# nerfstudio-project/nerfstudio

Measured on AMD Instinct MI355X. Metric: training rays/sec (4096 rays x 48 samples per GPU), higher is better.
Workload: dtype f32

## Files before the change

nerfstudio_amd/csrc/field_mlp.hip:

```cpp

#include "common.h"
#include "field_reduce.h"
#include "launch.h"
#include "mfma_chain.h"
#include "scatter.h"
#include "wave.h"

NSAMD_PROBE_DEFINE(field)

namespace nsamd {

constexpr int kWaves = 4;
constexpr int kFieldThreads = 64 * kWaves;
constexpr int kScratchLd = 20;
constexpr int kScratchTile = 64 * kScratchLd;

template <int NT, int KT, int THREADS>
__device__ __forceinline__ void stage_frag_load(float* v, const float* __restrict__ W, int n_real, int k_real, bool head0,
                                                int app_dim) {
  static_assert(THREADS % 256 == 0 && (NT * KT * 256) % THREADS == 0, "whole tiles per pass");
  const int r = threadIdx.x & 3, lane = (threadIdx.x >> 2) & 63;
  const int j = lane & 15, g = lane >> 4;
#pragma unroll
  for (int i = 0; i < NT * KT * 256 / THREADS; ++i) {
// ... 135 lines not shown
  stage_frag_load<4, 2, THREADS>(v, mlp.base_W0, 64, 32, false, 0);
  stage_frag_load<1, 4, THREADS>(v + 2 * U, mlp.base_W1, 16, 64, false, 0);
  stage_frag_load<4, 4, THREADS>(v + 3 * U, mlp.head_W0, 64, 31 + app_dim, true, app_dim);
  stage_frag_load<4, 4, THREADS>(v + 7 * U, mlp.head_W1, 64, 64, false, 0);
  stage_frag_load<1, 4, THREADS>(v + 11 * U, mlp.head_W2, 3, 64, false, 0);
  stage_frag_store<4, 2, THREADS>(wf + kOffBase0, v);
  stage_frag_store<1, 4, THREADS>(wf + kOffBase1, v + 2 * U);
  stage_frag_store<4, 4, THREADS>(wf + kOffHead0, v + 3 * U);
  stage_frag_store<4, 4, THREADS>(wf + kOffHead1, v + 7 * U);
  stage_frag_store<1, 4, THREADS>(wf + kOffHead2, v + 11 * U);
  stage_bias<THREADS>(bias + kBiasBase0, mlp.base_b0, 64, 64);
  stage_bias<THREADS>(bias + kBiasBase1, mlp.base_b1, 16, 16);
  stage_bias<THREADS>(bias + kBiasHead0, mlp.head_b0, 64, 64);
  stage_bias<THREADS>(bias + kBiasHead1, mlp.head_b1, 64, 64);
  stage_bias<THREADS>(bias + kBiasHead2, mlp.head_b2, 3, 16);
}

template <int WAVES, bool RAYC = false>
__global__ __launch_bounds__(64 * WAVES, WAVES == 16 ? 1 : 2) void field_mlp_fwd_kernel(
    const float* __restrict__ enc, const float* __restrict__ selector, const float* __restrict__ directions,
    const int64_t* __restrict__ cams, const float* __restrict__ app_const, int64_t dir_group, int64_t M,
    nsamd_field_mlp mlp, int app_dim, float* __restrict__ density, float* __restrict__ rgb) {
  extern __shared__ __attribute__((aligned(16))) float lds[];
  float* wf = lds;
  float* bias = lds + kFragTotal;
  PROBE_STAMP(WAVES, 0);
  stage_all_fwd<64 * WAVES>(wf, bias, mlp, app_dim);
  __syncthreads();
  PROBE_STAMP(WAVES, 1);
  const int lane = threadIdx.x & 63, wave = threadIdx.x >> 6;
  const int64_t tiles = (M + 15) / 16;
  const float* app_table = cams ? mlp.appearance : nullptr;
  int probe_it = 0;
  for (int64_t tile = (int64_t)blockIdx.x * WAVES + wave; tile < tiles; tile += (int64_t)gridDim.x * WAVES) {
    asm volatile("" ::: "memory");
    const TileInputs ti = tile_inputs(tile, lane, M, selector, cams, dir_group);
    FieldActs A;
    load_enc_tile_fwd(enc, M, ti.p, lane, A.enc);
    if (RAYC && rgb != nullptr) {
      const float* c = mlp.ray_terms + ti.ray * 64 + 4 * (lane >> 4);
#pragma unroll
      for (int n = 0; n < 4; ++n) A.ha[n] = *reinterpret_cast<const v4f*>(c + 16 * n);
    }
    PROBE_STAMP(WAVES, 2 + 4 * probe_it);
    field_forward_tile<RAYC>(wf, bias, directions, app_table, app_const, dir_group, M, app_dim, ti, lane, A, 3 + 4 * probe_it,
                             rgb == nullptr);
    PROBE_STAMP(WAVES, 4 + 4 * probe_it);
    if (rgb != nullptr && mlp.saved_hb != nullptr && ti.live) {
#pragma unroll
      for (int t = 0; t < 4; ++t) *reinterpret_cast<v4f*>(mlp.saved_hb + ((tile * 4 + t) * 64 + lane) * 4) = A.hb[t];
    }
    if (lane < 16 && ti.live) {
      density[ti.p] = mlp.average_init_density * expf(A.o16[0][0]) * ti.sel;
      if (rgb != nullptr) {
        float* o = rgb + 3 * ti.p;
#pragma unroll
        for (int c = 0; c < 3; ++c) o[c] = 1.0f / (1.0f + expf(-A.rgbp[0][c]));
      }
    }
    PROBE_STAMP(WAVES, 5 + 4 * probe_it);
    ++probe_it;
  }
  PROBE_STAMP(WAVES, 63);
}

__global__ __launch_bounds__(kFieldThreads) void field_ray_terms_kernel(
    const float* __restrict__ directions, const int64_t* __restrict__ cams, const float* __restrict__ app_const,
    int64_t num_rays, nsamd_field_mlp mlp, int app_dim, float* __restrict__ terms, float* __restrict__ inputs,
    const float* __restrict__ slot_dev, int32_t slots) {
  __shared__ __attribute__((aligned(16))) float wf[kFragHead0];
  __shared__ __attribute__((aligned(16))) float bias[64];
  if (slot_dev != nullptr) {
    int32_t slot = (int32_t)slot_dev[0];
    slot = slot < 0 ? 0 : (slot >= slots ? slots - 1 : slot);
    directions += (int64_t)slot * 3 * num_rays;
    if (cams != nullptr) cams += (int64_t)slot * num_rays;
  }
  {
    float v[16];
    stage_frag_load<4, 4, kFieldThreads>(v, mlp.head_W0, 64, 31 + app_dim, true, app_dim);
    stage_frag_store<4, 4, kFieldThreads>(wf, v);
    stage_bias<kFieldThreads>(bias, mlp.head_b0, 64, 64);
  }
  __syncthreads();
  const int lane = threadIdx.x & 63, wave = threadIdx.x >> 6;
  const int j = lane & 15, g = lane >> 4;
  const float* app_table = cams ? mlp.appearance : nullptr;
  const int64_t tiles = (num_rays + 15) / 16;
  for (int64_t tile = (int64_t)blockIdx.x * kWaves + wave; tile < tiles; tile += (int64_t)gridDim.x * kWaves) {
    const int64_t ray = tile * 16 + j;
    const bool live = ray < num_rays;
    const int64_t rc = live ? ray : num_rays - 1;
    const float* d = directions + 3 * rc;
    v4f hin[4];
    hin[0] = sh_quad(d[0], d[1], d[2], g);
    if (app_dim > 0) {
      const float* src = (app_table != nullptr) ? app_table + cams[rc] * 32 : app_const;
      hin[2] = *reinterpret_cast<const v4f*>(src + 4 * g);
      hin[3] = *reinterpret_cast<const v4f*>(src + 16 + 4 * g);
    } else {
      hin[2] = v4f{0.f, 0.f, 0.f, 0.f};
      hin[3] = v4f{0.f, 0.f, 0.f, 0.f};
    }
    v4f acc[4];
    load_bias<4>(bias, acc, g);
    chain_gemm_tile<4, 4>(wf, 0, hin[0], acc, lane);
    chain_gemm_tile<4, 4>(wf, 2, hin[2], acc, lane);
    chain_gemm_tile<4, 4>(wf, 3, hin[3], acc, lane);
    if (live) {
#pragma unroll
      for (int n = 0; n < 4; ++n) *reinterpret_cast<v4f*>(terms + ray * 64 + 16 * n + 4 * g) = acc[n];
      if (inputs != nullptr) {
        float* x = inputs + ray * (16 + app_dim);
        *reinterpret_cast<v4f*>(x + 4 * g) = hin[0];
        if (app_dim > 0) {
          *reinterpret_cast<v4f*>(x + 16 + 4 * g) = hin[2];
          *reinterpret_cast<v4f*>(x + 32 + 4 * g) = hin[3];
        }
      }
    }
  }
}

typedef __bf16 bf16x8 __attribute__((ext_vector_type(8)));
typedef __bf16 bf16x2 __attribute__((ext_vector_type(2)));
typedef unsigned u4 __attribute__((ext_vector_type(4)));

__device__ __forceinline__ v4f mfma_bf16(const u4& a, const u4& b, v4f c) {
  return __builtin_amdgcn_mfma_f32_16x16x32_bf16(__builtin_bit_cast(bf16x8, a), __builtin_bit_cast(bf16x8, b), c, 0, 0, 0);
}

__device__ __forceinline__ unsigned pack_bf16(float a, float b) {
  bf16x2 p;
  p[0] = (__bf16)a;
  p[1] = (__bf16)b;
  return __builtin_bit_cast(unsigned, p);
}

__global__ void probe_mfma_bf16_kernel(const float* __restrict__ A, const float* __restrict__ B, float* __restrict__ out) {
  const int lane = threadIdx.x, j = lane & 15, g = lane >> 4;
  u4 a, b;
#pragma unroll
  for (int q = 0; q < 4; ++q) {
    a[q] = pack_bf16(A[j * 32 + 8 * g + 2 * q], A[j * 32 + 8 * g + 2 * q + 1]);
    b[q] = pack_bf16(B[(8 * g + 2 * q) * 16 + j], B[(8 * g + 2 * q + 1) * 16 + j]);
  }
  v4f c = {0.f, 0.f, 0.f, 0.f};
  c = mfma_bf16(a, b, c);
#pragma unroll
  for (int r = 0; r < 4; ++r) out[(4 * g + r) * 16 + j] = c[r];
}

__device__ __forceinline__ void split_pair(float x0, float x1, unsigned& o0, unsigned& o1) {
  const unsigned hh = pack_bf16(x0, x1);
  const float r0 = x0 - __uint_as_float(hh << 16);
  const float r1 = x1 - __uint_as_float(hh & 0xffff0000u);
  o0 = pack_bf16(r0, x0);
  o1 = pack_bf16(r1, x1);
}

template <int T>
__device__ __forceinline__ void store_rows_f32(float* S, const v4f* x, int j, int g) {
#pragma unroll
  for (int t = 0; t < T; ++t)
#pragma unroll
    for (int r = 0; r < 4; ++r) S[(16 * t + 4 * g + r) * kScratchLd + j] = x[t][r];
}

template <int T>
__device__ __forceinline__ void store_rows_pk(float* S, const v4f* x, int j, int g) {
  unsigned* U = reinterpret_cast<unsigned*>(S);
#pragma unroll
  for (int t = 0; t < T; ++t)
#pragma unroll
    for (int r = 0; r < 4; r += 2) {
      unsigned o0, o1;
      split_pair(x[t][r], x[t][r + 1], o0, o1);
      U[(16 * t + 4 * g + r) * kScratchLd + j] = o0;
      U[(16 * t + 4 * g + r + 1) * kScratchLd + j] = o1;
    }
}

template <int NT>
__device__ __forceinline__ void relu_mask(v4f* grad, const v4f* act) {
#pragma unroll
  for (int n = 0; n < NT; ++n)
#pragma unroll
    for (int r = 0; r < 4; ++r) grad[n][r] = (act[n][r] > 0.0f) ? grad[n][r] : 0.0f;
}

constexpr int kRayS = 16 * kScratchLd, kRayX = kRayS + 64;
constexpr int kCoopWaves = 8;
constexpr int kCoopThreads = 64 * kCoopWaves;
constexpr int kLd64 = 68, kLd32 = 36;
constexpr int kRowBase0 = 0, kRowBase1 = kRowBase0 + 64 * kLd32, kRowHead0 = kRowBase1 + 16 * kLd64,
              kRowHead1 = kRowHead0 + 64 * kLd64, kRowHead2 = kRowHead1 + 64 * kLd64,
              kRowTotal = kRowHead2 + 16 * kLd64;

template <int N_PAD, int K_PAD>
__device__ __forceinline__ void stage_rows_load(float* v, const float* __restrict__ W, int n_real, int k_real, bool head0,
                                                int app_dim) {
#pragma unroll
  for (int i = 0; i < N_PAD * K_PAD / kCoopThreads; ++i) {
    const int e = threadIdx.x + i * kCoopThreads;
    const int row = e / K_PAD, slot = e % K_PAD;
    const int col = head0 ? head0_col(slot, app_dim) : slot;
    v[i] = (row < n_real && col >= 0 && col < k_real) ? W[row * k_real + col] : 0.0f;
  }
}

template <int N_PAD, int K_PAD, int LD>
__device__ __forceinline__ void stage_rows_store(float* dst, const float* v) {
#pragma unroll
  for (int i = 0; i < N_PAD * K_PAD / kCoopThreads; ++i) {
    const int e = threadIdx.x + i * kCoopThreads;
    dst[(e / K_PAD) * LD + e % K_PAD] = v[i];
  }
}

template <int NT, int KT, int LD>
__device__ __forceinline__ void rows_gemm_fwd(const float* Wrows, const v4f* in, v4f* out, int j, int g) {
#pragma unroll
  for (int t = 0; t < KT; ++t) {
    v4f a[NT];
#pragma unroll
    for (int n = 0; n < NT; ++n) a[n] = *reinterpret_cast<const v4f*>(Wrows + (16 * n + j) * LD + 16 * t + 4 * g);
#pragma unroll
    for (int r = 0; r < 4; ++r) {
#pragma unroll
      for (int n = 0; n < NT; ++n) out[n] = mfma16(a[n][r], in[t][r], out[n]);
    }
  }
}

template <int MT, int NT, int LD>
__device__ __forceinline__ void rows_gemm_bwd(const float* Wrows, const v4f* in, v4f* out, int j, int g) {
#pragma unroll
  for (int t = 0; t < NT; ++t) {
    float a[4][MT];
#pragma unroll
    for (int r = 0; r < 4; ++r)
#pragma unroll
      for (int m = 0; m < MT; ++m) a[r][m] = Wrows[(16 * t + 4 * g + r) * LD + 16 * m + j];
#pragma unroll
    for (int r = 0; r < 4; ++r)
#pragma unroll
      for (int m = 0; m < MT; ++m) out[m] = mfma16(a[r][m], in[t][r], out[m]);
  }
}

template <int MT, int LD>
__device__ __forceinline__ void rows_gemm_bwd_rgb(const float* Wrows, float in_k, v4f* out, int j, int g) {
  float a[MT];
#pragma unroll
  for (int m = 0; m < MT; ++m) a[m] = Wrows[g * LD + 16 * m + j];
#pragma unroll
  for (int m = 0; m < MT; ++m) out[m] = mfma16(a[m], in_k, out[m]);
}

struct NoBetween {
  template <int I>
  __device__ __forceinline__ void at() const {}
};

template <class Between = NoBetween, bool RAYC = false, bool SAVED = false>
__device__ __forceinline__ void coop_forward_tile(const float* W, const float* bias, const float (&dir)[3],
                                                  const float* __restrict__ app_table,
                                                  const float* __restrict__ app_const, int app_dim,
                                                  const TileInputs& ti, int lane, FieldActs& A, const v4f* app_pre = nullptr,
                                                  const Between& between = Between(), const v4f* ray_terms = nullptr) {
  const int j = lane & 15, g = lane >> 4;
  load_bias<4>(bias + kBiasBase0, A.h1, g);
  rows_gemm_fwd<4, 2, kLd32>(W + kRowBase0, A.enc, A.h1, j, g);
  if (SAVED) {
    asm volatile("" : "+v"(A.hb[0]), "+v"(A.hb[1]), "+v"(A.hb[2]), "+v"(A.hb[3]), "+v"(A.sg[0]), "+v"(A.sg[1]), "+v"(A.sg[2]));
  }
  between.template at<0>();
  relu_tiles<4>(A.h1);
  load_bias<1>(bias + kBiasBase1, A.o16, g);
  rows_gemm_fwd<1, 4, kLd64>(W + kRowBase1, A.h1, A.o16, j, g);
  between.template at<1>();
  if (RAYC) {
#pragma unroll
    for (int n = 0; n < 4; ++n) A.ha[n] = ray_terms[n];
    rows_gemm_fwd<4, 1, kLd64>(W + kRowHead0 + 16, A.o16, A.ha, j, g);
  } else {
  A.hin[0] = sh_quad(dir[0], dir[1], dir[2], g);
  A.hin[1] = A.o16[0];
  if (app_pre != nullptr) {
    A.hin[2] = app_pre[0];
    A.hin[3] = app_pre[1];
  } else if (app_dim > 0) {
    const float* src = (app_table != nullptr) ? app_table + ti.cam * 32 : app_const;
    A.hin[2] = *reinterpret_cast<const v4f*>(src + 4 * g);
    A.hin[3] = *reinterpret_cast<const v4f*>(src + 16 + 4 * g);
  } else {
    A.hin[2] = v4f{0.f, 0.f, 0.f, 0.f};
    A.hin[3] = v4f{0.f, 0.f, 0.f, 0.f};
  }
  load_bias<4>(bias + kBiasHead0, A.ha, g);
  rows_gemm_fwd<4, 4, kLd64>(W + kRowHead0, A.hin, A.ha, j, g);
  }
  between.template at<2>();
  relu_tiles<4>(A.ha);
  if (!SAVED) {
    load_bias<4>(bias + kBiasHead1, A.hb, g);
    rows_gemm_fwd<4, 4, kLd64>(W + kRowHead1, A.ha, A.hb, j, g);
  }
  between.template at<3>();
  if (!SAVED) {
    relu_tiles<4>(A.hb);
    load_bias<1>(bias + kBiasHead2, A.rgbp, g);
    rows_gemm_fwd<1, 4, kLd64>(W + kRowHead2, A.hb, A.rgbp, j, g);
  }
  between.template at<4>();
}

__device__ __forceinline__ float dot2_ones(unsigned a, float c) {
  asm("v_dot2c_f32_bf16 %0, %1, %2" : "+v"(c) : "v"(a), "v"(0x3f803f80u));
  return c;
}

template <int TILES>
__device__ __forceinline__ void coop_dw_f32(v4f* acc, float* dbacc, bool want_db, const float* scratch, int first,
                                            int count, int n, int m0, int j, int g) {
#pragma unroll 2
  for (int area = first; area < first + count; ++area) {
    const float* Sd = scratch + area * 2 * kScratchTile;
    const float* Sx = Sd + kScratchTile;
    const v4f a = *reinterpret_cast<const v4f*>(Sd + (16 * n + j) * kScratchLd + 4 * g);
    v4f b[TILES];
#pragma unroll
    for (int i = 0; i < TILES; ++i) b[i] = *reinterpret_cast<const v4f*>(Sx + (16 * (m0 + i) + j) * kScratchLd + 4 * g);
    if (want_db) *dbacc += (a[0] + a[1]) + (a[2] + a[3]);
#pragma unroll
    for (int q = 0; q < 4; ++q)
#pragma unroll
      for (int i = 0; i < TILES; ++i) acc[i] = mfma16(a[q], b[i][q], acc[i]);
  }
}

template <int TILES>
__device__ __forceinline__ void coop_dw_pk(v4f* acc, float* dbacc, bool want_db, const float* scratch, int first,
                                           int count, int n, int m0, int j, int g) {
#pragma unroll 2
  for (int area = first; area < first + count; ++area) {
    const float* Sd = scratch + area * 2 * kScratchTile;
    const float* Sx = Sd + kScratchTile;
    const u4 a = *reinterpret_cast<const u4*>(Sd + (16 * n + j) * kScratchLd + 4 * g);
    u4 b[TILES];
#pragma unroll
    for (int i = 0; i < TILES; ++i) b[i] = *reinterpret_cast<const u4*>(Sx + (16 * (m0 + i) + j) * kScratchLd + 4 * g);
    if (want_db) {
      float s = *dbacc;
#pragma unroll
      for (int q = 0; q < 4; ++q) s = dot2_ones(a[q], s);
      *dbacc = s;
    }
    u4 ar;
#pragma unroll
    for (int q = 0; q < 4; ++q) ar[q] = __builtin_amdgcn_alignbit(a[q], a[q], 16);
#pragma unroll
    for (int i = 0; i < TILES; ++i) acc[i] = mfma_bf16(a, b[i], acc[i]);
#pragma unroll
    for (int i = 0; i < TILES; ++i) acc[i] = mfma_bf16(ar, b[i], acc[i]);
  }
}

template <int T, bool HEAD0 = false>
__device__ __forceinline__ void store_rows(float* S, const v4f* x, int j, int g) {
  if (HEAD0) store_rows_f32<T>(S, x, j, g);
  else store_rows_pk<T>(S, x, j, g);
}

template <int TILES, bool HEAD0 = false>
__device__ __forceinline__ void coop_dw(v4f* acc, float* dbacc, bool want_db, const float* scratch, int first,
                                        int count, int n, int m0, int j, int g) {
  if (HEAD0) coop_dw_f32<TILES>(acc, dbacc, want_db, scratch, first, count, n, m0, j, g);
  else coop_dw_pk<TILES>(acc, dbacc, want_db, scratch, first, count, n, m0, j, g);
}

__device__ __forceinline__ void coop_emit(const v4f& acc, int n, int m, int k_pad, float* partial_layer,
                                          float* __restrict__ dst, int n_real, int k_real, bool head0, int app_dim,
                                          int j, int g) {
#pragma unroll
  for (int r = 0; r < 4; ++r) {
    const int row = 16 * n + 4 * g + r, slot = 16 * m + j;
    if (partial_layer != nullptr) {
      partial_layer[row * k_pad + slot] = acc[r];
    } else if (dst != nullptr) {
      const int col = head0 ? head0_col(slot, app_dim) : slot;
      if (row < n_real && col >= 0 && col < k_real) unsafeAtomicAdd(dst + row * k_real + col, acc[r]);
    }
  }
}

__device__ __forceinline__ void coop_emit_bias(float v, int n, int j, int g, float* partial_bias, float* __restrict__ dst,
                                               int n_real) {
  v += __shfl_xor(v, 16);
  v += __shfl_xor(v, 32);
  if (g == 0) {
    if (partial_bias != nullptr) partial_bias[16 * n + j] = v;
    else if (dst != nullptr && 16 * n + j < n_real) unsafeAtomicAdd(dst + 16 * n + j, v);
  }
}


struct RouteArgs {
  nsamd_points P;
  int transform;
  nsamd_aabb box;
  nsamd_grid grid;
  ScatterGeom G;
  ScatterBufs buf;
};

constexpr int kProducerSegCap = 256;
constexpr int kRouteLevels = 16;
constexpr int kRouteCnt = kRouteLevels * (1 << kProducerMaxLog2Bins);

struct RouteLds {
  uint32_t cnt[kRouteCnt];
  struct Level {
    float scal;
    uint32_t loff;
    uint32_t lmax;
    uint32_t pad;
  } lv[kRouteLevels];
  nsamd_points P;
  nsamd_aabb box;
  int32_t transform, num_levels, log2_table_size, slice_log2, log2_bins;
  uint32_t seg_cap, static_end, level_cap, spill_cap, segs;
  uint4* queues;
  uint32_t* dyn_cursor;
  uint32_t* hdr;
  uint4* spill_rec;
  uint32_t* spill_tile;
  uint32_t* counts;
  float stash[kCoopWaves][11][64];
};
constexpr int kRouteLdsWords = (sizeof(RouteLds) + 3) / 4;
static_assert(sizeof(float) * (kRowTotal + 256 + kCoopWaves * 2 * kScratchTile) + sizeof(RouteLds) <= 160 * 1024, "160 KiB of LDS per CU");

__device__ __forceinline__ void route_lds_init(RouteLds* L, const RouteArgs& R) {
  for (int e = threadIdx.x; e < kRouteCnt; e += kCoopThreads) L->cnt[e] = 0u;
  if (threadIdx.x < kRouteLevels) {
    L->lv[threadIdx.x].scal = R.grid.scalings[threadIdx.x];
    L->lv[threadIdx.x].loff = R.G.level_off[threadIdx.x];
    L->lv[threadIdx.x].lmax = 0u;
    L->lv[threadIdx.x].pad = 0u;
  }
  if (threadIdx.x == 0) {
    L->P = R.P;
    L->box = R.box;
    L->transform = R.transform;
    L->num_levels = R.grid.num_levels;
    L->log2_table_size = R.grid.log2_table_size;
    L->slice_log2 = R.G.slice_log2;
    L->log2_bins = R.G.log2_bins;
    L->seg_cap = R.G.seg_cap;
    L->static_end = R.G.segs * R.G.seg_cap;
    L->level_cap = R.G.level_cap[0];
    L->spill_cap = R.G.spill_cap;
    L->segs = R.G.segs;
    L->queues = R.buf.queues;
    L->dyn_cursor = R.buf.dyn_cursor;
    L->hdr = R.buf.hdr;
    L->spill_rec = R.buf.spill_rec;
    L->spill_tile = R.buf.spill_tile;
    L->counts = R.buf.counts;
  }
}

__device__ __forceinline__ void route_spill(RouteLds* L, uint32_t tile, uint4 rec) {
  const uint32_t pos = atomicAdd(L->hdr + kHdrSpillCount, 1u);
  if (pos < L->spill_cap) {
    L->spill_rec[pos] = rec;
    L->spill_tile[pos] = tile;
  } else {
    atomicAdd(L->hdr + kHdrEvtLost, 1u);
  }
}


__device__ __noinline__ void route_record_slow(RouteLds* L, float x, float y, float z, float g0, float g1, int level, int q,
                                               bool segment_full) {
  const uint32_t mask = (1u << L->log2_table_size) - 1u;
  const int sl = L->slice_log2, lb = L->log2_bins;
  const uint32_t local_mask = (1u << sl) - 1u;
  const Cell c = locate_cell(x, y, z, L->lv[level].scal);
  const PairHash h = pair_hash(c, q, mask);
  const uint32_t bin = h.ia >> sl, tile0 = (uint32_t)level << lb;
  float a0, a1;
  pair_share(c, q, g0, g1, a0, a1);
  if ((h.ib >> sl) != bin) {
    const float omx = 1.0f - c.w[0];
    route_spill(L, tile0 + bin, single_record(a0 * omx, a1 * omx, h.ia & local_mask));
    route_spill(L, tile0 + (h.ib >> sl), single_record(a0 * c.w[0], a1 * c.w[0], h.ib & local_mask));
    return;
  }
  if (!segment_full) return;
  const uint4 rec = pair_record(a0, a1, c.w[0], h.ia & local_mask, h.ib & local_mask);
  const uint32_t Q = L->level_cap, static_end = L->static_end;
  const uint32_t pos = atomicAdd(L->dyn_cursor + (tile0 + bin), 1u);
  if (pos < Q - static_end) rec_store(L->queues + (L->lv[level].loff + bin * Q + static_end + pos), rec);
  else route_spill(L, tile0 + bin, rec);
}

template <int K>
__device__ __forceinline__ void route_level(RouteLds* L, const float (*stash)[64], int lane, uint32_t& gmax) {
  constexpr int t = K >> 1, rr = K & 1;
  const int g = lane >> 4;
  const int level = 8 * t + 2 * g + rr;
  const float g0 = stash[4 * t + 2 * rr][lane], g1 = stash[4 * t + 2 * rr + 1][lane];
  if (level >= L->num_levels || (g0 == 0.0f && g1 == 0.0f)) return;
  const float x = stash[8][lane], y = stash[9][lane], z = stash[10][lane];
  const Cell c = locate_cell(x, y, z, L->lv[level].scal);
  {
    const uint32_t b0 = __float_as_uint(g0) & 0x7fffffffu, b1 = __float_as_uint(g1) & 0x7fffffffu;
    gmax = max(gmax, max(b0, b1));
  }
  const uint32_t mask = (1u << L->log2_table_size) - 1u;
  const int sl = L->slice_log2;
  const uint32_t local_mask = (1u << sl) - 1u;
  const uint32_t C = L->seg_cap;
  uint32_t* const cnt = L->cnt + ((uint32_t)level << L->log2_bins);
  PairHash h[4];
  uint32_t rank[4];
#pragma unroll
  for (int q = 0; q < 4; ++q) h[q] = pair_hash(c, q, mask);
#pragma unroll
  for (int q = 0; q < 4; ++q)
    rank[q] = atomicAdd(cnt + (h[q].ia >> sl), 1u);
  uint4* const base = L->queues + (L->lv[level].loff + blockIdx.x * C);
  const uint32_t level_cap = L->level_cap;
  bool slow[4], full[4];
#pragma unroll
  for (int q = 0; q < 4; ++q) {
    const uint32_t bin = h[q].ia >> sl;
    const bool straddle = (h[q].ib >> sl) != bin;
    const float bz = (q & 2) ? c.w[2] : 1.0f - c.w[2];
    const float by = (q & 1) ? c.w[1] : 1.0f - c.w[1];
    const uint32_t a0 = straddle ? 0u : __float_as_uint((g0 * bz) * by), a1 = straddle ? 0u : __float_as_uint((g1 * bz) * by);
    const uint4 rec = pair_record(__uint_as_float(a0), __uint_as_float(a1), c.w[0], h[q].ia & local_mask,
                                  (straddle ? h[q].ia : h[q].ib) & local_mask);
    full[q] = rank[q] >= C;
    slow[q] = straddle || full[q];
    if (!full[q]) rec_store(base + (bin * level_cap + rank[q]), rec);
    full[q] = full[q] && !straddle;
  }
#pragma unroll
  for (int q = 0; q < 4; ++q)
    if (slow[q]) route_record_slow(L, x, y, z, g0, g1, level, q, full[q]);
}

__device__ __forceinline__ void route_flush(RouteLds* L, const float (*stash)[64], int lane, uint32_t (&gmax)[4]) {
  route_level<0>(L, stash, lane, gmax[0]);
  route_level<1>(L, stash, lane, gmax[1]);
  route_level<2>(L, stash, lane, gmax[2]);
  route_level<3>(L, stash, lane, gmax[3]);
}

__device__ __forceinline__ void route_publish_max(RouteLds* L, int lane, const uint32_t (&gmax)[4]) {
#pragma unroll
  for (int K = 0; K < 4; ++K) {
    const int level = 8 * (K >> 1) + 2 * (lane >> 4) + (K & 1);
    const uint32_t m = row16_max_u32(gmax[K]);
    if ((lane & 15) == 0 && level < L->num_levels && m != 0u) atomicMax(&L->lv[level].lmax, m);
  }
}

struct RawPosition {
  float o[3], d[3], t0, t1;
};

__device__ __forceinline__ bool route_ray_layout(const RouteLds* L, int64_t dir_group) {
  return L->P.positions == nullptr && (int64_t)L->P.samples_per_ray == dir_group;
}

__device__ __forceinline__ void route_issue_position(const RouteLds* L, int64_t tile, int64_t tiles, int64_t M,
                                                     int64_t dir_group, int lane, RawPosition& rp) {
  const int64_t pt = tile * 16 + (lane & 15);
  const bool rays = route_ray_layout(L, dir_group) && tile < tiles && pt < M;
  const int64_t p = rays ? pt : 0;
  const int64_t S = dir_group, ray = point_ray(p, S), s = p - ray * S;
  const NSAMD_GLOBAL_AS float* dummy = global_ptr(reinterpret_cast<const float*>(L->hdr));
  const NSAMD_GLOBAL_AS float* tb = rays ? global_ptr(L->P.t_bins) + ray * (S + 1) + s : dummy;
  const NSAMD_GLOBAL_AS float* o = rays ? global_ptr(L->P.origins) + 3 * ray : dummy;
  const NSAMD_GLOBAL_AS float* d = rays ? global_ptr(L->P.directions) + 3 * ray : dummy;
  rp.o[0] = o[0], rp.o[1] = o[1], rp.o[2] = o[2];
  rp.d[0] = d[0], rp.d[1] = d[1], rp.d[2] = d[2];
  rp.t0 = tb[0], rp.t1 = tb[1];
}

__device__ __forceinline__ bool route_finish_position(const RouteLds* L, const RawPosition& rp, int64_t tile, int64_t tiles,
                                                      int64_t M, int64_t dir_group, int lane, float& x, float& y, float& z) {
  const int64_t p = tile * 16 + (lane & 15);
  x = y = z = 0.0f;
  if (!(tile < tiles && p < M)) return false;
  if (!route_ray_layout(L, dir_group)) {
    load_position(L->P, p, x, y, z);
  } else {
    const float span = rp.t0 + rp.t1;
    x = rp.o[0] + rp.d[0] * span / 2.0f;
    y = rp.o[1] + rp.d[1] * span / 2.0f;
    z = rp.o[2] + rp.d[2] * span / 2.0f;
  }
  return true;
}

struct TileFetch {
  TileInputs ti;
  v4f enc[2];
  float up[4];
  float dir[3];
  v4f app[2];
  v4f cterm[4];
  float xin;
};

template <bool RAYC = false>
__device__ __forceinline__ void fetch_tile(TileFetch& f, int64_t tile, int64_t tiles, int lane, int64_t M,
                                           const float* __restrict__ enc, const float* __restrict__ selector,
                                           const float* __restrict__ directions, const int64_t* __restrict__ cams,
                                           const float* __restrict__ app_table, const float* __restrict__ app_const,
                                           int app_dim, int64_t dir_group, const float* __restrict__ ddensity,
                                           const float* __restrict__ drgb, const float* __restrict__ ray_terms = nullptr,
                                           const float* __restrict__ ray_inputs = nullptr) {
  const int g = lane >> 4;
  const int64_t t = tile < tiles ? tile : tiles - 1;
  const int64_t p = t * 16 + (lane & 15);
  f.ti.live = p < M && tile < tiles;
  f.ti.p = p < M ? p : M - 1;
  f.ti.ray = point_ray(f.ti.p, dir_group);
  if (RAYC) {
    f.ti.cam = 0;
  } else {
    const int64_t* cam_src = cams != nullptr ? cams + f.ti.ray : reinterpret_cast<const int64_t*>(enc);
    f.ti.cam = *cam_src;
  }
  f.ti.sel = (selector != nullptr ? selector : enc)[f.ti.p];
  load_enc_tile(enc, M, f.ti.p, lane, f.enc);
#define NSAMD_KEEP_APART() asm volatile("" ::: "memory")
  f.up[0] = drgb[3 * f.ti.p + 0];
  NSAMD_KEEP_APART();
  f.up[1] = drgb[3 * f.ti.p + 1];
  NSAMD_KEEP_APART();
  f.up[2] = drgb[3 * f.ti.p + 2];
  NSAMD_KEEP_APART();
  f.up[3] = ddensity[f.ti.p];
  if (RAYC) {
    const float* c = ray_terms + f.ti.ray * 64 + 4 * g;
#pragma unroll
    for (int n = 0; n < 4; ++n) f.cterm[n] = *reinterpret_cast<const v4f*>(c + 16 * n);
    const int ncols = 16 + app_dim;
    f.xin = ray_inputs[f.ti.ray * ncols + (lane < ncols ? lane : 0)];
    return;
  }
  const float* d = directions + 3 * f.ti.ray;
  f.dir[0] = d[0];
  NSAMD_KEEP_APART();
  f.dir[1] = d[1];
  NSAMD_KEEP_APART();
  f.dir[2] = d[2];
  NSAMD_KEEP_APART();
  const float* src = app_table != nullptr ? app_table + (cams != nullptr ? f.ti.cam : 0) * 32
                                          : (app_const != nullptr ? app_const : enc);
  f.app[0] = *reinterpret_cast<const v4f*>(src + 4 * g);
  f.app[1] = *reinterpret_cast<const v4f*>(src + 16 + 4 * g);
#undef NSAMD_KEEP_APART
}

struct RouteBetween {
  RouteLds* L;
  const float (*stash)[64];
  int lane;
  bool on;
  uint32_t* gmax;
  template <int I>
  __device__ __forceinline__ void at() const {
    if (!on) return;
    if (I == 0) route_level<0>(L, stash, lane, gmax[0]);
    if (I == 2) route_level<1>(L, stash, lane, gmax[1]);
  }
};

template <bool ROUTE, bool RAYC = false, bool SAVED = false>
__global__ __launch_bounds__(kCoopThreads) void field_mlp_bwd_kernel(
    const float* __restrict__ enc, const float* __restrict__ selector, const float* __restrict__ directions,
    const int64_t* __restrict__ cams, const float* __restrict__ app_const, int64_t dir_group, int64_t M,
    nsamd_field_mlp mlp, int app_dim, const float* __restrict__ ddensity, const float* __restrict__ drgb,
    float* __restrict__ denc, nsamd_field_mlp_grads grads, float* __restrict__ partials,
    float* __restrict__ app_partials, int app_rows_per_point, RouteArgs R) {
  extern __shared__ __attribute__((aligned(16))) float lds[];
  float* W = lds;
  float* bias = lds + kRowTotal;
  float* scratch = bias + 256;
  RouteLds* RL = reinterpret_cast<RouteLds*>(scratch + kCoopWaves * 2 * kScratchTile);
  if (ROUTE) route_lds_init(RL, R);
  PROBE_STAMP(kCoopWaves, 0);
  {
    float v[24];
    stage_rows_load<64, 32>(v, mlp.base_W0, 64, 32, false, 0);
    stage_rows_load<16, 64>(v + 4, mlp.base_W1, 16, 64, false, 0);
    stage_rows_load<64, 64>(v + 6, mlp.head_W0, 64, 31 + app_dim, true, app_dim);
    stage_rows_load<64, 64>(v + 14, mlp.head_W1, 64, 64, false, 0);
    stage_rows_load<16, 64>(v + 22, mlp.head_W2, 3, 64, false, 0);
    stage_rows_store<64, 32, kLd32>(W + kRowBase0, v);
    stage_rows_store<16, 64, kLd64>(W + kRowBase1, v + 4);
    stage_rows_store<64, 64, kLd64>(W + kRowHead0, v + 6);
    stage_rows_store<64, 64, kLd64>(W + kRowHead1, v + 14);
    stage_rows_store<16, 64, kLd64>(W + kRowHead2, v + 22);
  }
  for (int e = threadIdx.x; e < 256; e += kCoopThreads) {
    float v = 0.0f;
    if (e < kBiasBase1) v = mlp.base_b0[e];
    else if (e < kBiasHead0) v = mlp.base_b1[e - kBiasBase1];
    else if (e < kBiasHead1) v = mlp.head_b0[e - kBiasHead0];
    else if (e < kBiasHead2) v = mlp.head_b1[e - kBiasHead1];
    else if (e < kBiasHead2 + 3) v = mlp.head_b2[e - kBiasHead2];
    bias[e] = v;
  }
  __syncthreads();

  const int lane = threadIdx.x & 63, wave = threadIdx.x >> 6;
  const int j = lane & 15, g = lane >> 4;
  float* Sd = scratch + wave * 2 * kScratchTile;
  float* Sx = Sd + kScratchTile;
  const float* app_table = cams ? mlp.appearance : nullptr;
  const int own_n = wave >> 1;
  const int own_m2 = 2 * (wave & 1);
  const int own_m1 = wave & 1;
  const int own_q = wave & 3;
  const int own_half = wave >> 2;
  v4f dW_h1[2], dW_h0[2], dW_b0[1], dW_h2[1], dW_b1[1];
  v4f dW_r[2];
  zero_tiles<2>(dW_r);
  float db_h1 = 0.f, db_h0 = 0.f, db_b0 = 0.f, db_h2 = 0.f, db_b1 = 0.f;
// ... 50 lines not shown
    const bool emit = ROUTE && it > 0;
#define NSAMD_ROUTE_LEVEL(K)                                                      \
  do {                                                                           \
    if (ROUTE) {                                                                 \
      if (emit) route_level<K>(RL, RL->stash[wave], lane, route_gmax[K]); \
    }                                                                            \
  } while (0)

    v4f g_rgbp[1];
    zero_tiles<1>(g_rgbp);
    if (g == 0 && ti.live) {
#pragma unroll
      for (int c = 0; c < 3; ++c) {
        const float sg = SAVED ? A.sg[c] : 1.0f / (1.0f + expf(-A.rgbp[0][c]));
        g_rgbp[0][c] = up_rgb[c] * (sg * (1.0f - sg));
      }
    }
    float g_rgb_k;
    {
      const float s0 = __shfl(g_rgbp[0][0], j), s1 = __shfl(g_rgbp[0][1], j), s2 = __shfl(g_rgbp[0][2], j);
      g_rgb_k = g == 0 ? s0 : (g == 1 ? s1 : (g == 2 ? s2 : 0.0f));
    }
    __syncthreads();
    store_rows<1>(Sd, g_rgbp, j, g);
    store_rows<4>(Sx, A.hb, j, g);
    v4f g_hb[4];
    zero_tiles<4>(g_hb);
    rows_gemm_bwd_rgb<4, kLd64>(W + kRowHead2, g_rgb_k, g_hb, j, g);
    relu_mask<4>(g_hb, A.hb);
    __syncthreads();
    coop_dw<1>(dW_h2, &db_h2, bias_owner14, scratch, 4 * own_half, 4, 0, own_q, j, g);
    __syncthreads();
    PROBE_STAMP(kCoopWaves, 4 + 10 * (int)it);

    store_rows<4>(Sd, g_hb, j, g);
    store_rows<4>(Sx, A.ha, j, g);
    v4f g_ha[4];
    zero_tiles<4>(g_ha);
    rows_gemm_bwd<4, 4, kLd64>(W + kRowHead1, g_hb, g_ha, j, g);
    relu_mask<4>(g_ha, A.ha);
    NSAMD_ROUTE_LEVEL(2);
    __syncthreads();
    coop_dw<2>(dW_h1, &db_h1, bias_owner44, scratch, 0, kCoopWaves, own_n, own_m2, j, g);
    __syncthreads();
    PROBE_STAMP(kCoopWaves, 5 + 10 * (int)it);

    v4f g_hin[4];
    zero_tiles<4>(g_hin);
    if (RAYC) {
      store_rows<4>(Sd, g_ha, j, g);
      store_rows<1>(Sx, A.o16, j, g);
      rows_gemm_bwd<1, 4, kLd64>(W + kRowHead0 + 16, g_ha, g_hin + 1, j, g);
      float* Ss = Sx + kRayS;
#pragma unroll
      for (int n = 0; n < 4; ++n) {
        v4f v = g_ha[n];
#pragma unroll
        for (int r = 0; r < 4; ++r) v[r] = row16_sum_lane0(v[r]);
        if (j == 0) *reinterpret_cast<v4f*>(Ss + 16 * n + 4 * g) = v;
      }
      if (lane < 48) Sx[kRayX + lane] = lane < 16 + app_dim ? nxt_xin : 0.0f;
      __syncthreads();
      {
        coop_dw<1>(dW_h0, &db_h0, true, scratch, 4 * own_half, 4, own_q, 0, j, g);
        const int a = wave & 3, b0 = wave >> 2;
#pragma unroll
        for (int h = 0; h < 2; ++h) {
          const float* area = scratch + (4 * h + g) * 2 * kScratchTile + kScratchTile;
          const float sa = area[kRayS + 16 * a + j];
          if (b0 == 0 || app_dim > 0) dW_r[0] = mfma16(sa, area[kRayX + 16 * b0 + j], dW_r[0]);
          if (wave < 4 && app_dim > 0) dW_r[1] = mfma16(sa, area[kRayX + 32 + j], dW_r[1]);
        }
        if (wave < 2 && app_partials != nullptr) {
          v4f o = {0.f, 0.f, 0.f, 0.f};
          const float* st = scratch + (j & 7) * 2 * kScratchTile + kScratchTile + kRayS;
#pragma unroll
          for (int kk = 0; kk < 16; ++kk)
            o = mfma16(W[kRowHead0 + (4 * kk + g) * kLd64 + 32 + 16 * wave + j], st[4 * kk + g], o);
          const int64_t tj = (it * gridDim.x + blockIdx.x) * kCoopWaves + j;
          if (j < 8 && tj < tiles)
            *reinterpret_cast<v4f*>(app_partials + ((uint32_t)tj * 32u + (uint32_t)(16 * wave + 4 * g))) = o;
        }
      }
      __syncthreads();
    } else {
    store_rows<4, true>(Sd, g_ha, j, g);
    store_rows<4, true>(Sx, A.hin, j, g);
    rows_gemm_bwd<3, 4, kLd64>(W + kRowHead0 + 16, g_ha, g_hin + 1, j, g);
    __syncthreads();
    coop_dw<2, true>(dW_h0, &db_h0, bias_owner44, scratch, 0, kCoopWaves, own_n, own_m2, j, g);
    __syncthreads();
    }
    PROBE_STAMP(kCoopWaves, 6 + 10 * (int)it);

    if (!RAYC && app_table != nullptr && grads.appearance != nullptr) {
      if (app_partials != nullptr && app_rows_per_point) {
        if (ti.live) {
#pragma unroll
          for (int t = 2; t < 4; ++t)
            *reinterpret_cast<v4f*>(app_partials + ti.p * 32 + 16 * (t - 2) + 4 * g) = g_hin[t];
        }
      } else if (app_partials != nullptr) {
#pragma unroll
        for (int t = 2; t < 4; ++t) {
          v4f v = g_hin[t];
#pragma unroll
          for (int r = 0; r < 4; ++r) v[r] = row16_sum_lane0(v[r]);
          if (j == 0 && tile < tiles)
            *reinterpret_cast<v4f*>(app_partials + ((uint32_t)tile * 32u + (uint32_t)(16 * (t - 2) + 4 * g))) = v;
        }
      } else {
        const int cam32 = (int)ti.cam;
        const int cam0 = __shfl(cam32, 0);
        const bool uniform = __all(cam32 == cam0);
        if (uniform) {
#pragma unroll
          for (int t = 2; t < 4; ++t)
#pragma unroll
            for (int r = 0; r < 4; ++r) {
              const float v = row16_sum_lane0(g_hin[t][r]);
              if (j == 0 && v != 0.0f) unsafeAtomicAdd(grads.appearance + (int64_t)cam0 * 32 + 16 * (t - 2) + 4 * g + r, v);
            }
        } else if (ti.live) {
#pragma unroll
          for (int t = 2; t < 4; ++t)
#pragma unroll
            for (int r = 0; r < 4; ++r)
              unsafeAtomicAdd(grads.appearance + ti.cam * 32 + 16 * (t - 2) + 4 * g + r, g_hin[t][r]);
        }
      }
    }

    v4f g_o16[1];
    g_o16[0] = g_hin[1];
    if (g == 0) {
      const float pre = A.o16[0][0];
      g_o16[0][0] = ti.live ? up_density * ti.sel * mlp.average_init_density *
                                  expf(fminf(fmaxf(pre, -15.0f), 15.0f))
                            : 0.0f;
    }
    store_rows<1>(Sd, g_o16, j, g);
    store_rows<4>(Sx, A.h1, j, g);
    v4f g_h1[4];
    zero_tiles<4>(g_h1);
    rows_gemm_bwd<4, 1, kLd64>(W + kRowBase1, g_o16, g_h1, j, g);
    relu_mask<4>(g_h1, A.h1);
    NSAMD_ROUTE_LEVEL(3);
    __syncthreads();
    coop_dw<1>(dW_b1, &db_b1, bias_owner14, scratch, 4 * own_half, 4, 0, own_q, j, g);
    __syncthreads();
    PROBE_STAMP(kCoopWaves, 7 + 10 * (int)it);

    RawPosition rawpos;
    if (ROUTE) route_issue_position(RL, tile, tiles, M, dir_group, lane, rawpos);
    store_rows<4>(Sd, g_h1, j, g);
    store_rows<2>(Sx, A.enc, j, g);
    v4f g_enc[2];
    zero_tiles<2>(g_enc);
    rows_gemm_bwd<2, 4, kLd32>(W + kRowBase0, g_h1, g_enc, j, g);
    if (ti.live && denc != nullptr) {
#pragma unroll
      for (int t = 0; t < 2; ++t)
#pragma unroll
        for (int r = 0; r < 4; ++r) (denc + (int64_t)(16 * t + r) * M)[enc_lane_offset(M, ti.p, lane)] = g_enc[t][r];
    }
    if (ROUTE) {
      float px, py, pz;
      const bool plive = route_finish_position(RL, rawpos, tile, tiles, M, dir_group, lane, px, py, pz);
      (void)normalise_position(RL->transform, RL->box, px, py, pz);
#pragma unroll
      for (int t = 0; t < 2; ++t)
#pragma unroll
        for (int r = 0; r < 4; ++r) RL->stash[wave][4 * t + r][lane] = plive ? g_enc[t][r] : 0.0f;
      RL->stash[wave][8][lane] = px;
      RL->stash[wave][9][lane] = py;
      RL->stash[wave][10][lane] = pz;
    }
    __syncthreads();
    if (it + 1 < iters)
      fetch_tile<RAYC>(nxt, tile + per_iter, tiles, lane, M, enc, selector, directions, cams, app_table, app_const, app_dim,
                       dir_group, ddensity, drgb, mlp.ray_terms, mlp.ray_inputs);
    PROBE_STAMP(kCoopWaves, 9 + 10 * (int)it);
    coop_dw<1>(dW_b0, &db_b0, own_m1 == 0, scratch, 0, kCoopWaves, own_n, own_m1, j, g);
    PROBE_STAMP(kCoopWaves, 8 + 10 * (int)it);
#undef NSAMD_ROUTE_LEVEL
  }
  if (ROUTE && iters > 0) {
    route_flush(RL, RL->stash[wave], lane, route_gmax);
    route_publish_max(RL, lane, route_gmax);
  }
  PROBE_STAMP(kCoopWaves, 62);

  float* stash = scratch;
  __syncthreads();
  if (ROUTE) {
    const int B = 1 << RL->log2_bins;
    for (int e = threadIdx.x; e < RL->num_levels * B; e += kCoopThreads) {
      const uint32_t n = RL->cnt[e];
      RL->counts[(size_t)e * RL->segs + blockIdx.x] = n < RL->seg_cap ? n : RL->seg_cap;
    }
    if (threadIdx.x < (unsigned)RL->num_levels && RL->lv[threadIdx.x].lmax != 0u)
      atomicMax(RL->hdr + threadIdx.x, RL->lv[threadIdx.x].lmax);
  }
  if (own_half == 1) {
    *reinterpret_cast<v4f*>(stash + ((0 * 4 + own_q) * 64 + lane) * 4) = dW_h2[0];
    *reinterpret_cast<v4f*>(stash + ((1 * 4 + own_q) * 64 + lane) * 4) = dW_b1[0];
    if (bias_owner14) {
      stash[2048 + lane] = db_h2;
      stash[2048 + 64 + lane] = db_b1;
    }
    if (RAYC) {
      *reinterpret_cast<v4f*>(stash + 2304 + (own_q * 64 + lane) * 4) = dW_h0[0];
      stash[2304 + 1024 + own_q * 64 + lane] = db_h0;
    }
  }
  __syncthreads();
  float* prow = partials != nullptr ? partials + (size_t)blockIdx.x * kPartialStride : nullptr;
  float* pbias = prow != nullptr ? prow + kFragTotal : nullptr;
  if (prow != nullptr) {
    for (int e = kBiasTotal + threadIdx.x; e < 256; e += kCoopThreads) pbias[e] = 0.0f;
  }
  if (own_half == 0) {
    const v4f o_h2 = *reinterpret_cast<const v4f*>(stash + ((0 * 4 + own_q) * 64 + lane) * 4);
    const v4f o_b1 = *reinterpret_cast<const v4f*>(stash + ((1 * 4 + own_q) * 64 + lane) * 4);
#pragma unroll
    for (int r = 0; r < 4; ++r) { dW_h2[0][r] += o_h2[r]; dW_b1[0][r] += o_b1[r]; }
    coop_emit(dW_h2[0], 0, own_q, 64, prow ? prow + kOffHead2 : nullptr, grads.head_W2, 3, 64, false, 0, j, g);
    coop_emit(dW_b1[0], 0, own_q, 64, prow ? prow + kOffBase1 : nullptr, grads.base_W1, 16, 64, false, 0, j, g);
    if (bias_owner14) {
      coop_emit_bias(db_h2 + stash[2048 + lane], 0, j, g, pbias ? pbias + kBiasHead2 : nullptr, grads.head_b2, 3);
      coop_emit_bias(db_b1 + stash[2048 + 64 + lane], 0, j, g, pbias ? pbias + kBiasBase1 : nullptr, grads.base_b1, 16);
    }
    if (RAYC) {
      const v4f o_h0 = *reinterpret_cast<const v4f*>(stash + 2304 + (own_q * 64 + lane) * 4);
#pragma unroll
      for (int r = 0; r < 4; ++r) dW_h0[0][r] += o_h0[r];
      coop_emit(dW_h0[0], own_q, 1, 64, prow ? prow + kOffHead0 : nullptr, grads.head_W0, 64, 31 + app_dim, true, app_dim, j, g);
      coop_emit_bias(db_h0 + stash[2304 + 1024 + own_q * 64 + lane], own_q, j, g, pbias ? pbias + kBiasHead0 : nullptr,
                     grads.head_b0, 64);
    }
  }
#pragma unroll
  for (int i = 0; i < 2; ++i) {
    coop_emit(dW_h1[i], own_n, own_m2 + i, 64, prow ? prow + kOffHead1 : nullptr, grads.head_W1, 64, 64, false, 0, j, g);
    if (!RAYC)
      coop_emit(dW_h0[i], own_n, own_m2 + i, 64, prow ? prow + kOffHead0 : nullptr, grads.head_W0, 64, 31 + app_dim, true,
                app_dim, j, g);
  }
  if (RAYC) {
    coop_emit(dW_r[0], wave & 3, wave < 4 ? 0 : 2, 64, prow ? prow + kOffHead0 : nullptr, grads.head_W0, 64, 31 + app_dim, true,
              app_dim, j, g);
    if (wave < 4)
      coop_emit(dW_r[1], wave, 3, 64, prow ? prow + kOffHead0 : nullptr, grads.head_W0, 64, 31 + app_dim, true, app_dim, j, g);
  }
  coop_emit(dW_b0[0], own_n, own_m1, 32, prow ? prow + kOffBase0 : nullptr, grads.base_W0, 64, 32, false, 0, j, g);
  if (bias_owner44) {
    coop_emit_bias(db_h1, own_n, j, g, pbias ? pbias + kBiasHead1 : nullptr, grads.head_b1, 64);
    if (!RAYC) coop_emit_bias(db_h0, own_n, j, g, pbias ? pbias + kBiasHead0 : nullptr, grads.head_b0, 64);
  }
  if (own_m1 == 0) coop_emit_bias(db_b0, own_n, j, g, pbias ? pbias + kBiasBase0 : nullptr, grads.base_b0, 64);
  PROBE_STAMP(kCoopWaves, 63);
}

__global__ __launch_bounds__(kReduceThreads) void field_dw_reduce_kernel(const float* __restrict__ partials,
                                                                          int num_partials,
                                                                          nsamd_field_mlp_grads grads, int app_dim,
                                                                          const float* __restrict__ app_rows,
                                                                          const int64_t* __restrict__ cams,
                                                                          int64_t num_rays, int tiles_per_ray) {
  extern __shared__ __attribute__((aligned(16))) float red_lds[];
  field_dw_reduce_body(red_lds, (int)blockIdx.x, partials, num_partials, grads, app_dim, app_rows, cams, num_rays, tiles_per_ray);
}

__global__ void probe_mfma16_kernel(const float* __restrict__ A, const float* __restrict__ B,
                                    float* __restrict__ out) {
  const int lane = threadIdx.x, j = lane & 15, g = lane >> 4;
  v4f c = {0.f, 0.f, 0.f, 0.f};
  c = mfma16(A[j * 4 + g], B[g * 16 + j], c);
#pragma unroll
  for (int r = 0; r < 4; ++r) out[(4 * g + r) * 16 + j] = c[r];
}

}

using namespace nsamd;

static int field_app_dim(const nsamd_field_mlp& mlp, const int64_t* cams, const float* app_const, int* app_dim) {
  if (cams != nullptr) NSAMD_REQUIRE(mlp.appearance != nullptr && mlp.num_images > 0);
  *app_dim = (cams != nullptr || app_const != nullptr) ? 32 : 0;
  return NSAMD_OK;
}

static int field_common_checks(const float* enc, const float* directions, int64_t dir_group, int64_t M,
                               const nsamd_field_mlp& mlp, const int64_t* cams, const float* app_const, int* app_dim) {
  NSAMD_REQUIRE(M >= 0 && dir_group >= 1);
  if (M > kMaxFieldPoints) return NSAMD_ERR_UNSUPPORTED;
  NSAMD_REQUIRE(enc && directions);
  NSAMD_REQUIRE(mlp.base_W0 && mlp.base_b0 && mlp.base_W1 && mlp.base_b1 && mlp.head_W0 && mlp.head_b0 &&
                mlp.head_W1 && mlp.head_b1 && mlp.head_W2 && mlp.head_b2);
  return field_app_dim(mlp, cams, app_const, app_dim);
}

static unsigned field_blocks(int64_t tiles, int waves) {
  return (unsigned)min((int64_t)device_cus(), (tiles + waves - 1) / waves);
}

static unsigned field_bwd_blocks(int64_t M) { return field_blocks((M + 15) / 16, kCoopWaves); }
// ... 207 lines not shown
```

nerfstudio_amd/csrc/wave.h:

```cpp
#pragma once
#include <hip/hip_runtime.h>

namespace nsamd {

__device__ __forceinline__ int wave_index() { return (int)(threadIdx.x >> 6); }

template <int CTRL, int ROW_MASK>
__device__ __forceinline__ double dpp_move_f64(double v) {
  const unsigned long long b = (unsigned long long)__double_as_longlong(v);
  int lo = (int)(unsigned)(b & 0xffffffffull), hi = (int)(unsigned)(b >> 32);
  lo = __builtin_amdgcn_update_dpp(0, lo, CTRL, ROW_MASK, 0xf, true);
  hi = __builtin_amdgcn_update_dpp(0, hi, CTRL, ROW_MASK, 0xf, true);
  return __longlong_as_double((long long)(((unsigned long long)(unsigned)hi << 32) | (unsigned long long)(unsigned)lo));
}

__device__ __forceinline__ double wave_scan_inclusive_f64(double v) {
  v = v + dpp_move_f64<0x111, 0xf>(v);
  v = v + dpp_move_f64<0x112, 0xf>(v);
  v = v + dpp_move_f64<0x114, 0xf>(v);
  v = v + dpp_move_f64<0x118, 0xf>(v);
  v = v + dpp_move_f64<0x142, 0xa>(v);
  v = v + dpp_move_f64<0x143, 0xc>(v);
  return v;
}

__device__ __forceinline__ double wave_shift_up1_f64(double v) { return dpp_move_f64<0x138, 0xf>(v); }

template <int LANE>
__device__ __forceinline__ double wave_read_f64(double v) {
  const unsigned long long b = (unsigned long long)__double_as_longlong(v);
  const unsigned lo = (unsigned)__builtin_amdgcn_readlane((int)(unsigned)(b & 0xffffffffull), LANE);
  const unsigned hi = (unsigned)__builtin_amdgcn_readlane((int)(unsigned)(b >> 32), LANE);
  return __longlong_as_double((long long)(((unsigned long long)hi << 32) | (unsigned long long)lo));
}

template <int CTRL, int ROW_MASK>
__device__ __forceinline__ uint32_t dpp_move_u32(uint32_t v) {
  return (uint32_t)__builtin_amdgcn_update_dpp(0, (int)v, CTRL, ROW_MASK, 0xf, true);
}
__device__ __forceinline__ uint32_t wave_scan_inclusive_u32(uint32_t v) {
  v += dpp_move_u32<0x111, 0xf>(v);
  v += dpp_move_u32<0x112, 0xf>(v);
  v += dpp_move_u32<0x114, 0xf>(v);
  v += dpp_move_u32<0x118, 0xf>(v);
  v += dpp_move_u32<0x142, 0xa>(v);
  v += dpp_move_u32<0x143, 0xc>(v);
  return v;
}

__device__ __forceinline__ uint32_t row16_max_u32(uint32_t v) {
  v = max(v, dpp_move_u32<0xB1, 0xf>(v));
  v = max(v, dpp_move_u32<0x4E, 0xf>(v));
  v = max(v, dpp_move_u32<0x124, 0xf>(v));
  v = max(v, dpp_move_u32<0x128, 0xf>(v));
  return v;
}

__device__ __forceinline__ uint32_t pair_swap_u32(uint32_t v) {
  return (uint32_t)__builtin_amdgcn_update_dpp(0, (int)v, 0xB1, 0xf, 0xf, false);
}
__device__ __forceinline__ float pair_swap_f32(float v) { return __uint_as_float(pair_swap_u32(__float_as_uint(v))); }

template <int CTRL>
__device__ __forceinline__ float dpp_move_f32(float v) {
  return __uint_as_float((uint32_t)__builtin_amdgcn_update_dpp(0, (int)__float_as_uint(v), CTRL, 0xf, 0xf, false));
}
__device__ __forceinline__ float row16_sum_lane0(float v) {
  v += dpp_move_f32<0xB1>(v);
  v += dpp_move_f32<0x4E>(v);
  v += dpp_move_f32<0x12C>(v);
  v += dpp_move_f32<0x128>(v);
  return v;
}

}
```

Baseline: 6.980 million.

## Pack per-level routing params into LDS, reuse tile ray index, tweak DPP/bf16 split

Each level's routing parameters (level count, count offset, segment capacity, level capacity, table size, slice shift, queue base pointer) now sit in a 16-byte-aligned per-level LDS record. route_level reads them from one place instead of several scattered scalar fields and no longer recomputes the count offset or queue base. route_issue_position takes the ray index already computed for the tile instead of deriving it with point_ray, which removes a divide. Separately, an empty asm barrier is placed on the bf16 pack in split_pair, and dpp_move_f32 switches bound_ctrl to true, which changes how invalid source lanes behave in row16_sum_lane0 and could alter the reduction result.

```diff
diff --git a/nerfstudio_amd/csrc/field_mlp.hip b/nerfstudio_amd/csrc/field_mlp.hip
--- a/nerfstudio_amd/csrc/field_mlp.hip
+++ b/nerfstudio_amd/csrc/field_mlp.hip
@@ -311,7 +311,8 @@
 }
 
 __device__ __forceinline__ void split_pair(float x0, float x1, unsigned& o0, unsigned& o1) {
-  const unsigned hh = pack_bf16(x0, x1);
+  unsigned hh = pack_bf16(x0, x1);
+  asm("" : "+v"(hh));
   const float r0 = x0 - __uint_as_float(hh << 16);
   const float r1 = x1 - __uint_as_float(hh & 0xffff0000u);
   o0 = pack_bf16(r0, x0);
@@ -580,11 +581,15 @@
 
 struct RouteLds {
   uint32_t cnt[kRouteCnt];
-  struct Level {
+  struct alignas(16) Level {
     float scal;
     uint32_t loff;
     uint32_t lmax;
-    uint32_t pad;
+    uint32_t num_levels;
+    uint32_t cnt_off;
+    uint32_t seg_cap, level_cap;
+    int32_t log2_table_size, slice_log2;
+    uint4* base;
   } lv[kRouteLevels];
   nsamd_points P;
   nsamd_aabb box;
@@ -607,7 +612,13 @@
     L->lv[threadIdx.x].scal = R.grid.scalings[threadIdx.x];
     L->lv[threadIdx.x].loff = R.G.level_off[threadIdx.x];
     L->lv[threadIdx.x].lmax = 0u;
-    L->lv[threadIdx.x].pad = 0u;
+    L->lv[threadIdx.x].num_levels = (uint32_t)R.grid.num_levels;
+    L->lv[threadIdx.x].cnt_off = threadIdx.x << R.G.log2_bins;
+    L->lv[threadIdx.x].seg_cap = R.G.seg_cap;
+    L->lv[threadIdx.x].level_cap = R.G.level_cap[0];
+    L->lv[threadIdx.x].log2_table_size = R.grid.log2_table_size;
+    L->lv[threadIdx.x].slice_log2 = R.G.slice_log2;
+    L->lv[threadIdx.x].base = R.buf.queues + (R.G.level_off[threadIdx.x] + blockIdx.x * R.G.seg_cap);
   }
   if (threadIdx.x == 0) {
     L->P = R.P;
@@ -672,18 +683,19 @@
   const int g = lane >> 4;
   const int level = 8 * t + 2 * g + rr;
   const float g0 = stash[4 * t + 2 * rr][lane], g1 = stash[4 * t + 2 * rr + 1][lane];
-  if (level >= L->num_levels || (g0 == 0.0f && g1 == 0.0f)) return;
+  const RouteLds::Level& lv = L->lv[level];
+  if ((uint32_t)level >= lv.num_levels || (g0 == 0.0f && g1 == 0.0f)) return;
   const float x = stash[8][lane], y = stash[9][lane], z = stash[10][lane];
-  const Cell c = locate_cell(x, y, z, L->lv[level].scal);
+  const Cell c = locate_cell(x, y, z, lv.scal);
   {
     const uint32_t b0 = __float_as_uint(g0) & 0x7fffffffu, b1 = __float_as_uint(g1) & 0x7fffffffu;
     gmax = max(gmax, max(b0, b1));
   }
-  const uint32_t mask = (1u << L->log2_table_size) - 1u;
-  const int sl = L->slice_log2;
+  const uint32_t mask = (1u << lv.log2_table_size) - 1u;
+  const int sl = lv.slice_log2;
   const uint32_t local_mask = (1u << sl) - 1u;
-  const uint32_t C = L->seg_cap;
-  uint32_t* const cnt = L->cnt + ((uint32_t)level << L->log2_bins);
+  const uint32_t C = lv.seg_cap;
+  uint32_t* const cnt = L->cnt + lv.cnt_off;
   PairHash h[4];
   uint32_t rank[4];
 #pragma unroll
@@ -691,8 +703,8 @@
 #pragma unroll
   for (int q = 0; q < 4; ++q)
     rank[q] = atomicAdd(cnt + (h[q].ia >> sl), 1u);
-  uint4* const base = L->queues + (L->lv[level].loff + blockIdx.x * C);
-  const uint32_t level_cap = L->level_cap;
+  uint4* const base = lv.base;
+  const uint32_t level_cap = lv.level_cap;
   bool slow[4], full[4];
 #pragma unroll
   for (int q = 0; q < 4; ++q) {
@@ -738,11 +750,11 @@
 }
 
 __device__ __forceinline__ void route_issue_position(const RouteLds* L, int64_t tile, int64_t tiles, int64_t M,
-                                                     int64_t dir_group, int lane, RawPosition& rp) {
+                                                     int64_t dir_group, int lane, int64_t tile_ray, RawPosition& rp) {
   const int64_t pt = tile * 16 + (lane & 15);
   const bool rays = route_ray_layout(L, dir_group) && tile < tiles && pt < M;
   const int64_t p = rays ? pt : 0;
-  const int64_t S = dir_group, ray = point_ray(p, S), s = p - ray * S;
+  const int64_t S = dir_group, ray = rays ? tile_ray : 0, s = p - ray * S;
   const NSAMD_GLOBAL_AS float* dummy = global_ptr(reinterpret_cast<const float*>(L->hdr));
   const NSAMD_GLOBAL_AS float* tb = rays ? global_ptr(L->P.t_bins) + ray * (S + 1) + s : dummy;
   const NSAMD_GLOBAL_AS float* o = rays ? global_ptr(L->P.origins) + 3 * ray : dummy;
@@ -1099,7 +1111,7 @@
     PROBE_STAMP(kCoopWaves, 7 + 10 * (int)it);
 
     RawPosition rawpos;
-    if (ROUTE) route_issue_position(RL, tile, tiles, M, dir_group, lane, rawpos);
+    if (ROUTE) route_issue_position(RL, tile, tiles, M, dir_group, lane, ti.ray, rawpos);
     store_rows<4>(Sd, g_h1, j, g);
     store_rows<2>(Sx, A.enc, j, g);
     v4f g_enc[2];
diff --git a/nerfstudio_amd/csrc/wave.h b/nerfstudio_amd/csrc/wave.h
--- a/nerfstudio_amd/csrc/wave.h
+++ b/nerfstudio_amd/csrc/wave.h
@@ -63,7 +63,7 @@
 
 template <int CTRL>
 __device__ __forceinline__ float dpp_move_f32(float v) {
-  return __uint_as_float((uint32_t)__builtin_amdgcn_update_dpp(0, (int)__float_as_uint(v), CTRL, 0xf, 0xf, false));
+  return __uint_as_float((uint32_t)__builtin_amdgcn_update_dpp(0, (int)__float_as_uint(v), CTRL, 0xf, 0xf, true));
 }
 __device__ __forceinline__ float row16_sum_lane0(float v) {
   v += dpp_move_f32<0xB1>(v);
```

New measurement: 7.045 million (median of 6 runs). Within noise of the previous version (+0.9%).
